# schmidtjonathan/pnmol-experiments

Measured on AMD Instinct MI355X. Metric: filter steps/sec, 1D heat N=512 nu=2 (white-noise EK1 predict+update), higher is better.
Workload: dtype f64; 1 GPU; 1-D heat equation, N=512 mesh, IWP(nu=2) EK1, Dirichlet, dt=2^-7, one problem per GPU (kappa sweep), D=1536, m=514; steps_in_one_call=4975, valid=True, problems_per_gpu=1

## Files before the change

### pnmol-experiments_amd/csrc/pnmol_hip.hip

```cpp
#include <hip/hip_runtime.h>

#include <algorithm>
#include <chrono>
#include <cmath>
#include <cstdio>
#include <cstdlib>
#include <cstring>
#include <string>
#include <utility>
#include <atomic>
#include <vector>

#include "pnmol_hip.h"
#include "pnmol_internal.hpp"

namespace {

constexpr int NB = 32;
constexpr int TLD = NB + 1;
constexpr int MAXN = 4;
typedef double d4 __attribute__((ext_vector_type(4)));

struct IwpConsts {
    double A1[MAXN * MAXN];
    double Q1[MAXN * MAXN];
    double ts[MAXN];
};

struct MeasModel {
    const int* ell_col;
    const double* ell_val;
    int w, d, m, dp, mp;
    double c0, c1;
};

constexpr int HW = 4;

struct HRow {
    int idx[HW + 1];
    double cf[HW + 1];
};

__device__ __forceinline__ void h_row_load(const MeasModel& mm, int i, HRow& r) {
    r.idx[0] = (i < mm.d) ? mm.dp + i : 0;
    r.cf[0] = (i < mm.d) ? mm.c1 : 0.0;
#pragma unroll
    for (int e = 0; e < HW; ++e) {
        const int cidx = (e < mm.w) ? mm.ell_col[e * mm.mp + i] : -1;
        const double val = (e < mm.w) ? mm.ell_val[e * mm.mp + i] : 0.0;
        r.idx[e + 1] = cidx >= 0 ? cidx : 0;
        r.cf[e + 1] = cidx >= 0 ? mm.c0 * val : 0.0;
    }
}

template <typename XT>
__device__ __forceinline__ double h_row_dot(const MeasModel& mm, int i, const XT* x) {
    double v = 0.0;
    if (i < mm.d) v = mm.c1 * x[mm.dp + i];
    for (int e = 0; e < mm.w; ++e) {
        const int cidx = mm.ell_col[e * mm.mp + i];
        if (cidx >= 0) v += mm.c0 * mm.ell_val[e * mm.mp + i] * x[cidx];
    }
    return v;
}

template <int W, typename XT>
__device__ __forceinline__ double h_row_dot_w(const HRow& r, const XT* __restrict__ x) {
    double xv[W + 1];
#pragma unroll
    for (int e = 0; e <= W; ++e) xv[e] = x[r.idx[e]];
    double v = r.cf[0] * xv[0];
#pragma unroll
    for (int e = 1; e <= W; ++e) v += r.cf[e] * xv[e];
    return v;
}

struct RoleArgs {
    IwpConsts c;
    int dp;
    const double* min;
    double* mpred;
    const double* shift;
    double* G;
    double* zbuf;
    MeasModel mm;
    int* flags;
    int nflags;
};

template <int N>
__device__ __forceinline__ void predict_vectors(double* mpl, int tid, const IwpConsts& c, int dp, const double* __restrict__ min,
                                                double* __restrict__ mpred, const double* __restrict__ shift,
                                                double* __restrict__ G, double* __restrict__ zbuf, const MeasModel& mm,
                                                int* __restrict__ flags, int nflags) {
    const long Dp = (long)N * dp;
    for (int e = tid; e < nflags; e += 256) flags[e] = 0;
    for (int j = tid; j < dp; j += 256) {
// ... 1563 lines not shown
                            break;
                        }
                        __builtin_amdgcn_s_sleep(1);
                    }
                }
                __syncthreads();
                const long Dp = (long)RBW * NB;
                const long row0 = (I < zb ? (long)(I - CB) * NB : Dp + (long)(I - zb - 1) * NB) + 8 * w;
                const double* W = F + (long)ld * ld;
                SWEEP_STAMP(2);
                vecops_rowsR<8>(dd.va, W, ld, Dp, row0, row0 + 8, l);
            }
        }
        if (tid == 0 && L.dead) atomicMin(info, -2);
        SWEEP_STAMP(5);
        return;
    }

    SWEEP_STAMP(3);
    if (w == 2 && I > 0) {
        drain_vmem();
        if (l == 0) flag_st(frow + I, I);
        __hip_atomic_store(&L.pub, 1, __ATOMIC_RELAXED, __HIP_MEMORY_SCOPE_WORKGROUP);
    }
    diag4_factor<true>(accD, &L.d4, w, l, F + ((long)I * NB) * ld + (long)I * NB, ld, Linv + (long)I * NB * NB, info, I * NB,
                       L.sd, smax, nullptr, pivot_tolerance(lenient));
    if (w == 1) {
        drain_vmem();
        if (I > 0) {
            int spins = 0;
            while (__hip_atomic_load(&L.pub, __ATOMIC_RELAXED, __HIP_MEMORY_SCOPE_WORKGROUP) == 0 && ++spins < (1 << 24))
                __builtin_amdgcn_s_sleep(1);
        }
        if (l == 0) flag_st(fdiag + I, 1);
        SWEEP_STAMP_L(4);
    }
    if (tid == 0 && L.dead) atomicMin(info, -2);
    if constexpr (CHAINHELP) {
        const int H = CB - 1 - I;
        if (I < H - 1) {
            const double* Xh = F + ((long)H * NB + fr) * ld + 8 * fk;
            for (int t = I + 3; t < H; ++t) {
                const int kh = helper_share(H, t, CB);
                if (kh <= 0) continue;
                int* cl = claim + (long)H * CB + t;
                __syncthreads();
                if (tid == 0) {
                    int got = 0;
                    for (int spins = 0;; ++spins) {
                        if (flag_ld(cl) != 0) break;
                        if (flag_ld(frow + H) >= kh && flag_ld(frow + t) >= kh) {
                            got = atomicCAS(cl, 0, 1) == 0;
                            break;
                        }
                        if (spins > 4096 || flag_ld(fabort)) {
                            got = -1;
                            break;
                        }
                        __builtin_amdgcn_s_sleep(8);
                    }
                    L.seen[0] = got;
                }
                __syncthreads();
                const int got = L.seen[0];
                if (got < 0) break;
                if (got == 0) continue;
                ksplit_partial(L.sP[w], Xh, F + ((long)t * NB + fr) * ld + 8 * fk, 0, kh, ld, w, l);
                __syncthreads();
                double* hs = hs_scratch + ((long)H * CB + t) * NB * NB;
#pragma unroll
                for (int r = 0; r < 4; ++r)
                    wt_st(&hs[(wr * 16 + fk + 4 * r) * NB + colC],
                          (L.sP[0][offC + 4 * r * TLD] + L.sP[1][offC + 4 * r * TLD]) +
                              (L.sP[2][offC + 4 * r * TLD] + L.sP[3][offC + 4 * r * TLD]));
                drain_vmem();
                __syncthreads();
                if (tid == 0) flag_st(cl, 2);
            }
        }
    }
}

constexpr int RL_REP = 8;
constexpr int S_SPLIT_FROM = 11, S_SPLIT_H = 9;
__host__ __device__ inline int s_split_count(int CB, bool xl) { return (xl && CB > S_SPLIT_FROM) ? CB - S_SPLIT_FROM : 0; }
constexpr int W_SPLIT_H = 11;
#ifndef PNMOL_W_SPLIT
#define PNMOL_W_SPLIT 0
#endif
__host__ __device__ inline int w_split_count(int RT, int CB) {
    const int RBW = RT - 2 * CB - 1;
    return (PNMOL_W_SPLIT && RBW > 0 && CB > W_SPLIT_H + 1) ? RBW : 0;
}
struct RlFlags {
    int frow, fabort, fxcc, ffeed, fdiag, fnew, fcol, fdiagL, fnewL, frowL, CBp, total;
};
__host__ __device__ inline RlFlags rl_flags(int RT, int CB) {
    const int RTp = (RT + 31) / 32 * 32, CBp = (CB + 31) / 32 * 32;
    RlFlags f;
    f.CBp = CBp;
    f.frow = 0;
    f.fabort = RTp;
    f.fxcc = RTp + 16;
    f.ffeed = RTp + 32;
    f.fdiag = f.ffeed + CBp;
    f.fnew = f.fdiag + RL_REP * CBp;
    f.fcol = f.fnew + RL_REP * CBp;
    f.fdiagL = f.fcol + RL_REP * CBp;
    f.fnewL = f.fdiagL + CBp;
    f.frowL = f.fnewL + CBp;
    f.total = f.frowL + CBp;
    return f;
}
__device__ __forceinline__ int xcc_id() { return __builtin_amdgcn_s_getreg((3 << 11) | 20) & 15; }
struct WaveWait {
    bool dead;
};
__device__ __forceinline__ void wave_wait_ge(const int* p, int need, int* fabort, WaveWait& ww) {
    if (ww.dead) return;
    for (int spins = 0;; ++spins) {
        if (flag_ld(p) >= need) return;
        if (spins > SWEEP_SPIN_LIMIT || ((spins & 63) == 63 && flag_ld(fabort))) {
            ww.dead = true;
            flag_st(fabort, 1);
            return;
        }
        __builtin_amdgcn_s_sleep(1);
    }
}
__device__ __forceinline__ void relay_wait_ge(const int* p, int need, int* relay, int tag, int* fabort, WaveWait& ww, int w) {
    if (w == 0) {
        wave_wait_ge(p, need, fabort, ww);
        __hip_atomic_store(relay, ww.dead ? (1 << 30) : tag, __ATOMIC_RELAXED, __HIP_MEMORY_SCOPE_WORKGROUP);
    } else {
        int v;
        while ((v = __hip_atomic_load(relay, __ATOMIC_RELAXED, __HIP_MEMORY_SCOPE_WORKGROUP)) < tag) __builtin_amdgcn_s_sleep(1);
        if (v == (1 << 30)) ww.dead = true;
    }
    asm volatile("" ::: "memory");
}

template <class Need>
__device__ __forceinline__ void relay_progress(const int* p, int cnt, Need need, int want, int& known, int* relay, int* fabort,
                                               WaveWait& ww, int w, int l) {
    if (w == 0) {
        if (known < want) {
            for (int spins = 0; !ww.dead; ++spins) {
                const int v = l < cnt ? flag_ld(p + l) : 0;
                const unsigned long long ok = __ballot(l < cnt && v >= need(l));
                known = __builtin_amdgcn_readfirstlane((int)__builtin_ctzll(~ok));
                if (known >= want) break;
                if (spins > SWEEP_SPIN_LIMIT || ((spins & 63) == 63 && flag_ld(fabort))) {
                    ww.dead = true;
                    flag_st(fabort, 1);
                    break;
                }
                __builtin_amdgcn_s_sleep(1);
            }
            __hip_atomic_store(relay, ww.dead ? (1 << 30) : known, __ATOMIC_RELAXED, __HIP_MEMORY_SCOPE_WORKGROUP);
        }
    } else {
        int v;
        while ((v = __hip_atomic_load(relay, __ATOMIC_RELAXED, __HIP_MEMORY_SCOPE_WORKGROUP)) < want) __builtin_amdgcn_s_sleep(1);
        if (v == (1 << 30)) ww.dead = true;
    }
    asm volatile("" ::: "memory");
}
__device__ __forceinline__ void relay_progress_min(const int* p, int cnt, int want, int& known, int* relay, int* fabort,
                                                   WaveWait& ww, int w, int l) {
    if (w == 0) {
        if (known < want) {
            for (int spins = 0; !ww.dead; ++spins) {
                int v = l < cnt ? flag_ld(p + l) : (1 << 29);
#pragma unroll
                for (int o = 32; o > 0; o >>= 1) v = min(v, __shfl_xor(v, o));
                known = __builtin_amdgcn_readfirstlane(v);
// ... 170 lines not shown
        if (XL && w == 1 && J + 1 < CB) {
            TileRegs t1;
            tile_regs_from_lds(t1, C.sLinv, l);
            tile_regs_store<0>(t1, rlinv, (unsigned)(J * NB * NB * 8), NB, l);
            drain_vmem();
            if (l == 0) l2_flag_st(rflags, fl.fdiagL + J, 1);
        }
        if (J + 1 == CB) {
            __syncthreads();
            if (w == 2) {
                wt_rows_from_lds<8>(rlinv, (unsigned)(J * NB * NB * 8), NB, C.sLinv, 0, l);
                drain_vmem();
                if (l < RL_REP) flag_st(fdiag_all + l * CBp + J, 1);
                if (XL && l == 0) l2_flag_st(rflags, fl.fdiagL + J, 1);
            }
            break;
        }
        if (w == 0 || w == 2) {
            wave_wait_ge(ffeed + J + 1, 1, fabort, ww);
            sc1_tile_to_lds((w == 2) ? C.sFeedD : C.sFeedS, rfeed, (unsigned)((2 * (J + 1) + (w == 2 ? 1 : 0)) * NB * NB * 8), l);
            if (w == 2 && l < NB) C.sd[(J + 1) & 1][l] = G[(long)((J + 1) * NB + l) * ld + (J + 1) * NB + l];
        }
        __syncthreads();
        CHAIN_TRACE(J, 2);
        if (tid < 16) C.d4[(J + 1) & 1].flagA[tid] = 0;
        TileRegs tl;
        if (w == 2) {
            if constexpr (XL) {
                tile_regs_from_lds(tl, C.sLinv, l);
            } else {
                wt_rows_from_lds<8>(rlinv, (unsigned)(J * NB * NB * 8), NB, C.sLinv, 0, l);
            }
        }
        d4 x = {0, 0, 0, 0};
#pragma unroll
        for (int s = 0; s < 8; ++s)
            x = __builtin_amdgcn_mfma_f64_16x16x4f64(C.sFeedS[(wr * 16 + fr) * TLD + 8 * fk + s],
                                                     C.sLinv[(wc * 16 + fr) * TLD + 8 * fk + s], x, 0, 0, 0);
#pragma unroll
        for (int r = 0; r < 4; ++r) C.sX[offC + 4 * r * TLD] = x[r];
#pragma unroll
        for (int r = 0; r < 4; ++r) accD[r] = C.sFeedD[offC + 4 * r * TLD];
        __syncthreads();
        CHAIN_TRACE(J, 3);
        if (w == 2) {
            if constexpr (!XL) {
                drain_vmem();
                if (l < RL_REP) flag_st(fdiag_all + l * CBp + J, 1);
            }
        }
#pragma unroll
        for (int s = 0; s < 8; ++s)
            accD = __builtin_amdgcn_mfma_f64_16x16x4f64(C.sX[(wr * 16 + fr) * TLD + 8 * fk + s],
                                                        C.sX[(wc * 16 + fr) * TLD + 8 * fk + s], accD, 0, 0, 0);
        if (w == 2) {
            const unsigned orgX = (unsigned)((((long)(J + 1) * NB) * ld + (long)J * NB) * 8);
            if constexpr (XL) {
                TileRegs tx;
                tile_regs_from_lds(tx, C.sX, l);
                tile_regs_store<0>(tx, rF, orgX, ld, l);
                drain_vmem();
                if (l == 0) l2_flag_st(rflags, fl.fnewL + J, 1);
                tile_regs_store<16>(tl, rlinv, (unsigned)(J * NB * NB * 8), NB, l);
                tile_regs_store<16>(tx, rF, orgX, ld, l);
                drain_vmem();
                if (l < RL_REP) flag_st(fdiag_all + l * CBp + J, 1);
                if (l < RL_REP) flag_st(fnew_all + l * CBp + J, 1);
            } else {
                wt_rows_from_lds<8>(rF, orgX, ld, C.sX, 0, l);
                drain_vmem();
                if (l < RL_REP) flag_st(fnew_all + l * CBp + J, 1);
            }
        }
    }
    if (w == 2)
        diag4_output(&C.d4[(CB - 1) & 1], l, F + ((long)(CB - 1) * NB) * ld + (long)(CB - 1) * NB, ld, info, (CB - 1) * NB,
                     C.sd[(CB - 1) & 1], smax, pivtol);
    if (l == 0 && ww.dead) atomicMin(info, -2);
}

template <int N, bool FUSED, int MAXT, bool XL>
__global__ __launch_bounds__(256) void k_sweep_rl(const double* __restrict__ G, double* F, double* Linv, int ld, int CB,
                                                  int RT, int* flags, int* info_base, const int* __restrict__ ctr,
                                                  DowndateArgs dd, double* feed, int lenient, int home) {
    __shared__ __attribute__((aligned(16))) union {
        SweepLds L;
        ChainLds C;
    } lds;
    SweepLds& L = lds.L;
    __shared__ __attribute__((aligned(16))) double bulk_ring[4][RING + 2][16 * NB];
    const int tid = threadIdx.x, l = tid & 63, w = __builtin_amdgcn_readfirstlane(tid >> 6);
    const int wr = w >> 1, wc = w & 1, fr = l & 15, fk = l >> 4;
    const RlFlags fl = rl_flags(RT, CB);
    int* frow = flags + fl.frow;
    int* fabort = flags + fl.fabort;
    int* ffeed = flags + fl.ffeed;
    const int* fdiag = flags + fl.fdiag + (blockIdx.x % RL_REP) * fl.CBp;
    const int* fnew = flags + fl.fnew + (blockIdx.x % RL_REP) * fl.CBp;
    const int* fcol = flags + fl.fcol + (blockIdx.x % RL_REP) * fl.CBp;
    int* info = info_base + (*ctr - 1);
    const int bx = XL ? (int)blockIdx.x - home : (int)blockIdx.x;
    if (bx < 0) return;
    if (bx == 0) {
        sweep_chain_role<XL>(lds.C, G, F, Linv, ld, CB, flags, fl, info, feed, lenient, tid, l, w);
        return;
    }
    int I, part = 0;
    if constexpr (XL) {
        const int nsplit = s_split_count(CB, true);
        const int b = bx, nslot = 8 * (CB - 1 + nsplit) + 1;
        if (b < nslot) {
            if (b % 8 != 0) return;
            const int sidx = b / 8;
            if (sidx < CB) {
                I = sidx;
                part = (nsplit > 0 && I >= S_SPLIT_FROM) ? 1 : 0;
            } else {
                I = S_SPLIT_FROM + (sidx - CB);
                part = 2;
            }
        } else {
            if (b % 8 == 0) return;
            const int q = b - nslot;
            I = CB + q - (q + 1) / 8;
        }
    } else {
        I = bx - 1;
    }
#ifdef PNMOL_SWEEP_STAMP
    if (tid == 0) L.stamp_id = part == 1 ? 200 + I : 1 + I;
#endif
    {
        const int zb = RT - CB - 1;
        if (I >= CB && I <= zb) I = (I == CB) ? zb : I - 1;
    }
    const int nwsplit = w_split_count(RT, CB);
    if (I >= RT && I < RT + nwsplit) {
        I = CB + (I - RT);
        part = 2;
    } else if (I >= RT) {
        I -= nwsplit;
        if constexpr (FUSED) {
            if (tid == 0) {
                L.dead = 0, L.seen[0] = 0;
                __builtin_amdgcn_fence(__ATOMIC_ACQUIRE, "agent");
            }
            __syncthreads();
            SWEEP_STAMP(0);
            sweep_downdate_role<N, true>(L, dd, F, ld, CB, CB, frow, fabort, info, I - RT, tid, l, w, *ctr - 1);
        }
        return;
    } else if (nwsplit > 0 && I >= CB && I < RT - CB - 1) {
        part = 1;
    }
    const bool chain = I < CB;
    if (chain && I == 0) return;
    if (tid == 0) {
        L.dead = 0, L.pub = 0, L.pubcnt = part == 2 ? 4 * (I < CB ? S_SPLIT_H : W_SPLIT_H) : 0, L.rdiag = 0, L.rnew = 0, L.rcol = 0, L.rzb = 0;
        L.seen[0] = 0;
        __builtin_amdgcn_fence(__ATOMIC_ACQUIRE, "agent");
    }
    __syncthreads();
    SWEEP_STAMP(0);

    const long rowC = (long)I * NB + wr * 16 + fk;
    const int colC = wc * 16 + fr;
    const int offC = (wr * 16 + fk) * TLD + colC;
    const bool feeds = chain && part != 1;
    const int hsplit = chain ? S_SPLIT_H : W_SPLIT_H;
    const int t0 = part == 2 ? hsplit : 0;
    const int last = part == 1 ? hsplit - 1 : (chain ? I - 2 : CB - 1);
    const int ntiles = part == 1 ? hsplit : (chain ? I : CB);
    d4 n[MAXT];
#pragma unroll
    for (int t = 0; t < MAXT; ++t)
        if (t0 + t < ntiles) {
#pragma unroll
            for (int r = 0; r < 4; ++r) n[t][r] = -G[(rowC + 4 * r) * ld + (long)(t0 + t) * NB + colC];
        }
    d4 accD = {0, 0, 0, 0};
    if (feeds) {
#pragma unroll
        for (int r = 0; r < 4; ++r) {
            const int rl = wr * 16 + fk + 4 * r, cl = colC;
            accD[r] = -G[((long)I * NB + (rl >= cl ? rl : cl)) * ld + (long)I * NB + (rl >= cl ? cl : rl)];
        }
    }
    WaveWait ww{false};
    int known_diag = 0, known_new = 0, known_col = 0;
    const __amdgpu_buffer_rsrc_t rF = wt_rsrc(F), rfeed = wt_rsrc(feed), rflags = wt_rsrc(flags);
    const double* ringw = &bulk_ring[w][0][0];
    const unsigned ring0 = __builtin_amdgcn_readfirstlane((unsigned)(size_t)ringw);
    int roff[4], roffL[4];
#pragma unroll
    for (int c = 0; c < 4; ++c) {
        const int row = 4 * c + (l >> 4);
        roff[c] = (wc * 16 + row) * ld + 2 * ((l & 15) ^ row);
        roffL[c] = (wc * 16 + row) * NB + 2 * ((l & 15) ^ row);
    }
#ifndef PNMOL_EAGER_TILES
#define PNMOL_EAGER_TILES 6
#endif
    constexpr int EAGER_TILES = PNMOL_EAGER_TILES;
    bool pre_b0 = false;
    if constexpr (FUSED) {
        const int RBW = RT - 2 * CB - 1, zb = CB + RBW;
        if (!chain && I > zb) {
            double bq[8] = {0, 0, 0, 0, 0, 0, 0, 0};
            if (dd.va.Sqinv != nullptr) rows8_dot(dd.va.Sqinv, (long)(I - zb - 1) * NB + 8 * w, ld, dd.va.z, bq, l);
            if (l == 0) {
#pragma unroll
                for (int q = 0; q < 8; ++q) L.sd[8 * w + q] = bq[q];
            }
        }
    }
    bool local = false;
    if constexpr (XL) {
        if (chain) {
            if (tid == 0) {
                int v = 0;
                for (int spins = 0; spins < 4096 && (v = flag_ld(flags + fl.fxcc)) == 0; ++spins) __builtin_amdgcn_s_sleep(1);
                L.seen[0] = (v == 1 + xcc_id());
            }
            __syncthreads();
            local = L.seen[0] != 0;
            if (local) fdiag = flags + fl.fdiagL, fnew = flags + fl.fnewL;
        }
    }
    Frag8 ax;
    auto flag_tile = [&](int t) {
        drain_vmem();
        int lastw = 0;
        if (l == 0) lastw = __hip_atomic_fetch_add(&L.pubcnt, 1, __ATOMIC_RELAXED, __HIP_MEMORY_SCOPE_WORKGROUP) == 4 * t + 3;
        if (__builtin_amdgcn_readfirstlane(lastw)) {
            if (l == 0) flag_st(frow + I, t + 1);
            if (XL && chain && l == 0) {
                if (local) l2_flag_st(rflags, fl.frowL + I, t + 1);
                else flag_st(flags + fl.frowL + I, t + 1);
            }
            if (chain && l < RL_REP)
                __hip_atomic_fetch_add(flags + fl.fcol + l * fl.CBp + t, 1, __ATOMIC_RELAXED, __HIP_MEMORY_SCOPE_AGENT);
        }
    };
    if (part == 2) {
        const int* fsrc = (XL && local) ? flags + fl.frowL : frow;
        for (int k = 0; k < t0; ++k) {
            if (chain) {
                if (k + 1 < t0) {
                    relay_progress_min(fsrc + t0, I - t0 + 1, k + 1, known_col, &L.rcol, fabort, ww, w, l);
                } else {
                    relay_progress(fnew, CB - 1, [](int) { return 1; }, t0, known_new, &L.rnew, fabort, ww, w, l);
                    relay_progress_min(fsrc + t0 + 1, I - t0, t0, known_col, &L.rcol, fabort, ww, w, l);
                }
            } else {
                relay_progress(fnew, CB - 1, [](int) { return 1; }, k + 1, known_new, &L.rnew, fabort, ww, w, l);
                relay_progress(fcol, CB - 1, [CB](int q) { return CB - 2 - q; }, k + 1, known_col, &L.rcol, fabort, ww, w, l);
                relay_wait_ge(frow + I, k + 1, &L.rzb, k + 1, fabort, ww, w);
            }
            Frag8 bx;
            frag_ld(ax, F + ((long)I * NB + wr * 16 + fr) * ld + (long)k * NB + 8 * fk);
            frag_ld(bx, F + ((long)I * NB + wc * 16 + fr) * ld + (long)k * NB + 8 * fk);
#pragma unroll
            for (int u0 = 0; u0 < 8; u0 += 4) {
                Frag8 b[4];
#pragma unroll
                for (int q = 0; q < 4; ++q)
                    if (t0 + u0 + q < ntiles)
                        frag_ld(b[q], F + ((long)(t0 + u0 + q) * NB + wc * 16 + fr) * ld + (long)k * NB + 8 * fk);
#pragma unroll
                for (int q = 0; q < 4; ++q)
                    if (t0 + u0 + q < ntiles) {
#pragma unroll
                        for (int s = 0; s < 8; ++s)
                            n[u0 + q] = __builtin_amdgcn_mfma_f64_16x16x4f64(ax.v[s], b[q].v[s], n[u0 + q], 0, 0, 0);
                    }
            }
            if (chain) {
#pragma unroll
                for (int s = 0; s < 8; ++s) accD = __builtin_amdgcn_mfma_f64_16x16x4f64(ax.v[s], bx.v[s], accD, 0, 0, 0);
            }
            mfma_result_guard();
        }
    }
    const bool lastlocal = feeds && XL && local;
#pragma unroll
    for (int r = 0; r < 4; ++r) L.sS[t0 & 1][offC + 4 * r * TLD] = -n[0][r];
    __syncthreads();
    bool pre_l = false;
    for (int j = t0; j <= last; ++j) {
// ... 244 lines not shown
        }
#pragma unroll
        for (int a = 0; a < N; ++a) {
            st[(a * 16 + lr) * C::SLD + lc] = pa[a].x;
            st[(a * 16 + lr) * C::SLD + lc + 1] = pa[a].y;
            st[((N + a) * 16 + lr) * C::SLD + lc] = pb[a].x;
            st[((N + a) * 16 + lr) * C::SLD + lc + 1] = pb[a].y;
        }
        asm volatile("" ::: "memory");
        __builtin_amdgcn_wave_barrier();
#pragma unroll
        for (int kk = 0; kk < C::CW / 4; ++kk) {
            double fa[N], fb[N];
#pragma unroll
            for (int a = 0; a < N; ++a) {
                fa[a] = st[(a * 16 + fr) * C::SLD + kk * 4 + fk];
                fb[a] = st[((N + a) * 16 + fr) * C::SLD + kk * 4 + fk];
            }
#pragma unroll
            for (int a = 0; a < N; ++a)
#pragma unroll
                for (int b = 0; b < N; ++b)
                    acc[a][b] = __builtin_amdgcn_mfma_f64_16x16x4f64(fa[a], fb[b], acc[a][b], 0, 0, 0);
        }
        asm volatile("" ::: "memory");
        __builtin_amdgcn_wave_barrier();
    }
    __syncthreads();
    if (w >= 2) {
        double* rd = smem + (w - 2) * C::RED;
#pragma unroll
        for (int a = 0; a < N; ++a)
#pragma unroll
            for (int b = 0; b < N; ++b)
#pragma unroll
                for (int r = 0; r < 4; ++r) rd[((a * N + b) * 4 + r) * 64 + l] = acc[a][b][r];
    }
    __syncthreads();
    if (w >= 2) return;
    {
        const double* rd = smem + w * C::RED;
#pragma unroll
        for (int a = 0; a < N; ++a)
#pragma unroll
            for (int b = 0; b < N; ++b)
#pragma unroll
                for (int r = 0; r < 4; ++r) acc[a][b][r] += rd[((a * N + b) * 4 + r) * 64 + l];
    }
    __syncthreads();
    if (w == 0)
        downdate_finish<N, 0>(acc, smem, Ppred, Pout, var, dp, Dp, J, K, l);
    else
        downdate_finish<N, 1>(acc, smem, Ppred, Pout, var, dp, Dp, J, K, l);
}

__global__ __launch_bounds__(256) void k_fill_q(void* __restrict__ Qf, const double* __restrict__ Kg, IwpConsts c, int n,
                                                int dp, int p32) {
    const long Dp = (long)n * dp;
    const long e = (long)blockIdx.x * 256 + threadIdx.x;
    if (e >= Dp * Dp) return;
    const long row = e / Dp, col = e % Dp;
    const int a = (int)(row / dp), j = (int)(row % dp), b = (int)(col / dp), k = (int)(col % dp);
    const double v = c.Q1[a * MAXN + b] * Kg[(long)j * dp + k];
    if (p32) static_cast<float*>(Qf)[e] = (float)v;
    else static_cast<double*>(Qf)[e] = v;
}

__global__ __launch_bounds__(256) void k_ttt(const double* __restrict__ T, double* __restrict__ C, int mp) {
    __shared__ double sa[16][17], sb[16][17];
    const int tx = threadIdx.x & 15, ty = threadIdx.x >> 4;
    const int i = blockIdx.y * 16 + ty, k = blockIdx.x * 16 + tx;
    double acc = 0.0;
    for (int q0 = 0; q0 < mp; q0 += 16) {
        sa[ty][tx] = T[(long)(blockIdx.y * 16 + ty) * mp + q0 + tx];
        sb[ty][tx] = T[(long)(blockIdx.x * 16 + ty) * mp + q0 + tx];
        __syncthreads();
#pragma unroll
        for (int q = 0; q < 16; ++q) acc += sa[ty][q] * sb[tx][q];
        __syncthreads();
    }
    C[(long)i * mp + k] = acc;
}

template <int N, bool ROLE>
__global__ __launch_bounds__(256) void k_readout(const double* __restrict__ mean, const double* __restrict__ var,
                                                 double* __restrict__ means_base, double* __restrict__ stds_base,
                                                 double s0, int d, const double* __restrict__ part,
                                                 double* __restrict__ rec_base, int mp, int* __restrict__ ctr,
                                                 RoleArgs ra, int* __restrict__ tickets, int rblocks,
                                                 const void* __restrict__ Ppred, const double* __restrict__ rdiag,
                                                 const double* __restrict__ Rdense, int p32) {
    if constexpr (ROLE) {
        if ((int)blockIdx.x > rblocks) {
            const int fb = blockIdx.x - rblocks - 1;
            if (p32) front_block_tiled(static_cast<const float*>(Ppred), ra.G, rdiag, Rdense, ra.mm, (long)N * ra.dp, fb);
            else front_block_tiled(static_cast<const double*>(Ppred), ra.G, rdiag, Rdense, ra.mm, (long)N * ra.dp, fb);
            return;
        }
    }
    const int slot = __builtin_amdgcn_readfirstlane(*ctr) - 1;
    if constexpr (ROLE) {
        if ((int)blockIdx.x == rblocks) {
            extern __shared__ double mpl[];
            predict_vectors<N>(mpl, threadIdx.x, ra.c, ra.dp, ra.min, ra.mpred, ra.shift, ra.G, ra.zbuf, ra.mm, ra.flags,
                               ra.nflags);
            if (threadIdx.x == 0) {
                int spins = 0;
                while (__hip_atomic_load(tickets, __ATOMIC_RELAXED, __HIP_MEMORY_SCOPE_AGENT) < rblocks &&
                       ++spins < (1 << 22)) __builtin_amdgcn_s_sleep(1);
                *ctr = slot + 2;
                __hip_atomic_store(tickets, 0, __ATOMIC_RELAXED, __HIP_MEMORY_SCOPE_AGENT);
            }
            return;
        }
        __syncthreads();
        if (threadIdx.x == 0) atomicAdd(tickets, 1);
    }
    const int j = blockIdx.x * blockDim.x + threadIdx.x;
    double* means = means_base ? means_base + (size_t)slot * d : nullptr;
    double* stds = stds_base ? stds_base + (size_t)slot * d : nullptr;
    double* rec = rec_base + 4 * (size_t)slot;
    if (j < d) {
        if (means) means[j] = s0 * mean[j];
        if (stds) stds[j] = s0 * sqrt(fmax(var[j], 0.0));
    }
    if (blockIdx.x == 0) {
        __shared__ double sred[3][4];
        double a[3] = {0.0, 0.0, 0.0};
        for (int i = threadIdx.x; i < mp; i += 256)
#pragma unroll
            for (int q = 0; q < 3; ++q) a[q] += part[q * mp + i];
#pragma unroll
        for (int q = 0; q < 3; ++q)
#pragma unroll
            for (int o = 32; o > 0; o >>= 1) a[q] += __shfl_xor(a[q], o);
        if ((threadIdx.x & 63) == 0)
            for (int q = 0; q < 3; ++q) sred[q][threadIdx.x >> 6] = a[q];
        __syncthreads();
        if (threadIdx.x < 3) rec[threadIdx.x] = sred[threadIdx.x][0] + sred[threadIdx.x][1] + sred[threadIdx.x][2] + sred[threadIdx.x][3];
    }
}

__global__ __launch_bounds__(256) void k_poison(double* __restrict__ F, long nF, double* __restrict__ Linv, long nL,
                                                double* __restrict__ hs, long nH) {
    const double bad = __longlong_as_double(0x7ff8dead0000beefLL);
    const long stride = (long)gridDim.x * 256;
    for (long e = (long)blockIdx.x * 256 + threadIdx.x; e < nF; e += stride) F[e] = bad;
    for (long e = (long)blockIdx.x * 256 + threadIdx.x; e < nL; e += stride) {
        const int r = (int)((e / NB) % NB), c = (int)(e % NB);
        if (!(r < 16 && c >= 16)) Linv[e] = bad;
    }
    for (long e = (long)blockIdx.x * 256 + threadIdx.x; e < nH; e += stride) hs[e] = bad;
}

__global__ void k_operator_diagonal(double* __restrict__ ell_val, const double* __restrict__ base_val,
                                    const int* __restrict__ slot, const double* __restrict__ op ,
                                    double* __restrict__ shift, int d, int mp) {
    const int i = blockIdx.x * blockDim.x + threadIdx.x;
    if (i >= mp) return;
    if (i < d) {
        const int e = slot[i];
        ell_val[(long)e * mp + i] = base_val[(long)e * mp + i] - op[i];
    }
    shift[i] = op[d + i];
}

constexpr int FD_MAXS = 16;
__global__ __launch_bounds__(128) void k_fd_solve(const double* __restrict__ gram, const double* __restrict__ dk,
                                                  const double* __restrict__ llk, int N, int s, double* __restrict__ w,
                                                  double* __restrict__ unc) {
    const int p = blockIdx.x * blockDim.x + threadIdx.x;
    if (p >= N) return;
    double A[FD_MAXS][FD_MAXS], b[FD_MAXS];
    for (int i = 0; i < s; ++i) {
        for (int k = 0; k < s; ++k) A[i][k] = gram[((long)p * s + i) * s + k];
        b[i] = dk[(long)p * s + i];
    }
    for (int c = 0; c < s; ++c) {
        int piv = c;
        double best = fabs(A[c][c]);
        for (int i = c + 1; i < s; ++i)
            if (fabs(A[i][c]) > best) best = fabs(A[i][c]), piv = i;
        if (piv != c) {
            for (int k = 0; k < s; ++k) {
                const double t = A[c][k];
                A[c][k] = A[piv][k], A[piv][k] = t;
            }
            const double t = b[c];
            b[c] = b[piv], b[piv] = t;
        }
        const double inv = 1.0 / A[c][c];
        for (int i = c + 1; i < s; ++i) {
            const double f = A[i][c] * inv;
            A[i][c] = f;
            for (int k = c + 1; k < s; ++k) A[i][k] -= f * A[c][k];
        }
    }
    for (int i = 1; i < s; ++i)
        for (int k = 0; k < i; ++k) b[i] -= A[i][k] * b[k];
    for (int i = s - 1; i >= 0; --i) {
        for (int k = i + 1; k < s; ++k) b[i] -= A[i][k] * b[k];
        b[i] /= A[i][i];
    }
    double dot = 0.0;
    for (int i = 0; i < s; ++i) {
        w[(long)p * s + i] = b[i];
        dot += b[i] * dk[(long)p * s + i];
    }
    unc[p] = llk[p] - dot;
}

#define HIPCHK(ctx, call)                                                                        \
    do {                                                                                         \
        hipError_t e__ = (call);                                                                 \
// ... 206 lines not shown
    IwpConsts iwp{};
    int* ell_col = nullptr;
    double* ell_val = nullptr;
    int* ell_col_base = nullptr;
    double* ell_val_base = nullptr;
    int* ell_diag_slot = nullptr;
    int base_w = 0, base_has_diag = 0;
    int ell_is_base = 1;
    double* h_op = nullptr;
    double* h_op_dev = nullptr;
    hipEvent_t ev_op = nullptr;
    double *Kg = nullptr, *rdiag = nullptr, *Rdense = nullptr, *shift = nullptr;
    double *G = nullptr, *F = nullptr, *Linv = nullptr, *Ppred = nullptr, *mpred = nullptr, *zbuf = nullptr;
    double *var = nullptr, *Sqinv = nullptr, *rec = nullptr, *part = nullptr, *sdiag = nullptr;
    int* info = nullptr;
    std::vector<double> sqdiag;
    double* Qfull = nullptr;
    int* one = nullptr;
    int* info_err = nullptr;
    double sq_dt = -1.0;
    std::vector<double> hB;
    int ell_cap = 0;
    double *tmpP = nullptr, *tmpMean = nullptr;
    double *rec_means = nullptr, *rec_stds = nullptr;
    double* h_pin = nullptr;
    double* h_pin_dev = nullptr;
    int rec_cap = 0;
    hipEvent_t ev0 = nullptr, ev1 = nullptr;
    float last_ms = 0.f;
    int* ctr = nullptr;
    int pending_k = 0;
    double pending_dt = 0.0;
    pnmol_state* pending_state = nullptr;
    struct GraphEntry {
        double *P0, *P1, *var;
        double dt;
        int nsteps;
        bool have_sq;
        bool fused;
        hipGraphExec_t exec;
        bool launched;
    };
    std::vector<GraphEntry> graphs;
    int graph_chunk = 10;

};

struct pnmol_state {
    pnmol_filter* f = nullptr;
    double* mean = nullptr;
    double* P = nullptr;
    double* var = nullptr;
    double t = 0.0;
    double frame_dt = 0.0;
};

namespace {

void drop_graphs(pnmol_filter* f);

enum StepKind { STEP_FULL = 0, STEP_FIRST = 1, STEP_STEADY = 2 };

inline bool fused_loop(const pnmol_filter* f) { return f->sweep_mode == 2 && f->n <= 3 && f->fuse_predict != 0; }

inline bool sweep_rl_enabled() {
    static const int on = [] {
        const char* e = std::getenv("PNMOL_HIP_SWEEP_RL");
        return e ? std::atoi(e) : 1;
    }();
    return on != 0;
}
inline int sweep_xl_mode() {
    static const int mode = [] {
        const char* e = std::getenv("PNMOL_HIP_SWEEP_XL");
        return e ? (std::atoi(e) != 0 ? 1 : 0) : -1;
    }();
    return mode;
}
constexpr int MAX_DEVICES = 64;
std::atomic<int> live_rl_filters[MAX_DEVICES];
template <int N, bool FUSED>
void launch_sweep(unsigned grid, hipStream_t st, const double* G, double* F, double* Linv, int ld, int CB, int RT, int* flags,
                  int* info, const int* ctr, const DowndateArgs& dd, int* claim, double* hs, int lenient, int home,
                  bool wskip = false) {
    const bool xl = home >= 0;
    const unsigned rgrid = grid + (unsigned)w_split_count(RT, CB);
    unsigned xgrid = 8u * (unsigned)(CB - 1 + s_split_count(CB, true)) + 1u;
    for (unsigned left = rgrid - (unsigned)CB; left > 0; ++xgrid)
        if (xgrid % 8u != 0u) --left;
    xgrid += (unsigned)(xl ? home : 0);
    if (sweep_rl_enabled() && CB <= 9) {
        if (xl) k_sweep_rl<N, FUSED, 9, true><<<xgrid, 256, 0, st>>>(G, F, Linv, ld, CB, RT, flags, info, ctr, dd, hs, lenient, home);
        else k_sweep_rl<N, FUSED, 9, false><<<rgrid + 1, 256, 0, st>>>(G, F, Linv, ld, CB, RT, flags, info, ctr, dd, hs, lenient, home);
    } else if (sweep_rl_enabled() && CB <= 17) {
        if (xl) k_sweep_rl<N, FUSED, 17, true><<<xgrid, 256, 0, st>>>(G, F, Linv, ld, CB, RT, flags, info, ctr, dd, hs, lenient, home);
        else k_sweep_rl<N, FUSED, 17, false><<<rgrid + 1, 256, 0, st>>>(G, F, Linv, ld, CB, RT, flags, info, ctr, dd, hs, lenient, home);
    }
    else
        k_sweep<N, FUSED><<<grid, 256, 0, st>>>(G, F, Linv, ld, CB, RT, flags, info, ctr, dd, claim, hs, lenient, wskip ? 1 : 0);
}

inline bool short_last_panel() {
    static const int on = [] {
        const char* e = std::getenv("PNMOL_HIP_SHORT_LAST");
        return e ? std::atoi(e) : 1;
    }();
    return on != 0;
}
template <int N>
int launch_step(pnmol_filter* f, const double* Pin, const double* min, double frame_dt, double dt, double* Pout,
                double* mout, double* varout, bool record, StepKind kind) {
    pnmol_ctx* ctx = f->ctx;
    hipStream_t st = ctx->stream;
    IwpConsts c = f->iwp;
    for (int a = 0; a < f->n; ++a) {
        const double so = frame_dt == 0.0 ? 1.0 : nordsieck_scale(f->nu, a, frame_dt);
        c.ts[a] = so / nordsieck_scale(f->nu, a, dt);
    }
    MeasModel mm{f->ell_col, f->ell_val, f->ellw, f->d, f->m, f->dp, f->mp,
                 nordsieck_scale(f->nu, 0, dt), nordsieck_scale(f->nu, 1, dt)};
    const int dp = f->dp, mp = f->mp;
    const long Dp = f->Dp;

    if (kind != STEP_STEADY)
        k_predict<N><<<dim3(dp / 32, dp / 8 + 1), dim3(32, 8), sizeof(double) * Dp, st>>>(
        Pin, f->Ppred, f->Kg, c, dp, min, f->mpred, f->shift, f->G, f->zbuf, mm, f->ctr, f->flags, f->nflags, f->p32);
    if (kind != STEP_STEADY) {
        if (f->ellw > HW && f->sweep_mode != 0) {
            k_front<<<dim3((mp + 255) / 256, (unsigned)Dp), 256, 0, st>>>(f->Ppred, f->G, f->rdiag, f->Rdense, mm, Dp, f->p32);
            k_front_s<<<dim3((mp + 255) / 256, (unsigned)mp), 256, 0, st>>>(f->G, f->rdiag, f->Rdense, mm);
        } else {
            k_front<<<dim3((mp + 255) / 256, (unsigned)(Dp + mp + (f->sweep_mode == 0 ? mp : 0))), 256, 0, st>>>(
                f->Ppred, f->G, f->rdiag, f->Rdense, mm, Dp, f->p32);
        }
    }
    const long rowI0 = (long)mp + Dp + NB;
    const double* W = f->F + (long)mp * mp;
    const bool have_sq = (f->Sqinv != nullptr && f->sq_dt == dt);
    VecArgs va{f->mpred, f->F + ((long)mp + Dp) * mp, f->F + rowI0 * mp, f->zbuf, have_sq ? f->Sqinv : nullptr,
               mout, f->part};
    const int nreal = f->m - NB * (f->CB - 1);
    DowndateArgs dd{f->Ppred, Pout, varout, dp, 0, va, kind == STEP_FULL ? nullptr : f->Ppred, f->Kg, f->last_ctr, {}, {}, f->p32,
                    (nreal < 8 && short_last_panel()) ? nreal : 0};
    std::memcpy(dd.A1, f->iwp.A1, sizeof(dd.A1));
    std::memcpy(dd.Q1, f->iwp.Q1, sizeof(dd.Q1));
    if (f->sweep_mode == 2) {
        const int t32 = dp / NB, pairs = t32 * (t32 + 1) / 2;
        dd.vrows = 0;
        if constexpr (N <= 3)
            launch_sweep<N, true>(f->RT + pairs, st, f->G, f->F, f->Linv, mp, f->CB, f->RT, f->flags, f->info, f->ctr, dd,
                                  f->flags + f->RT + f->CB + 1, f->hs_scratch, f->p32 ? 2 : 0, f->xcd_home);
    } else {
        if (f->sweep_mode == 1) {
            if (f->w_gemm) {
                launch_sweep<N, false>(2 * f->CB + 1, st, f->G, f->F, f->Linv, mp, f->CB, f->RT, f->flags, f->info, f->ctr, dd,
                                       f->flags + f->RT + f->CB + 1, f->hs_scratch, f->p32 ? 2 : 0, f->xcd_home, true);
                const int nI = (int)(Dp / BDT), nt = nI * (mp / BDT);
                k_w_gemm<<<8 * ((nt + 7) / 8), 256, 0, st>>>(f->G + (long)mp * mp, f->F + rowI0 * mp, f->F + (long)mp * mp, mp, nI, nt);
            } else
            launch_sweep<N, false>(f->RT, st, f->G, f->F, f->Linv, mp, f->CB, f->RT, f->flags, f->info, f->ctr, dd,
                                   f->flags + f->RT + f->CB + 1, f->hs_scratch, f->p32 ? 2 : 0, f->xcd_home);
        } else {
            k_diag0<<<1, 128, 0, st>>>(f->G, f->F, f->Linv, mp, f->info, f->sdiag, f->ctr);
            for (int j = 0; j < f->CB; ++j) {
                const int nrb = f->RT - (j + 1);
                const int ncb = f->CB - 1 - j > 0 ? f->CB - 1 - j : 1;
                k_panel<<<dim3(nrb, ncb), 256, 0, st>>>(f->G, f->F, f->Linv, mp, j, f->CB, f->RBS, f->info, f->sdiag, f->ctr);
            }
        }
        const int tiles = dp / 16;
        const int vrows = (int)(((Dp + mp + 3) / 4 + tiles - 1) / tiles);
        if (f->dd_big) {
            const int T = (int)(Dp / BDT), nt = T * (T + 1) / 2;
            if (f->p32)
                k_downdate_big<float><<<8 * ((nt + 7) / 8), 256, 0, st>>>(reinterpret_cast<const float*>(f->Ppred), W,
                                                                          reinterpret_cast<float*>(Pout), varout, Dp, mp, nt);
            else
                k_downdate_big<double><<<8 * ((nt + 7) / 8), 256, 0, st>>>(static_cast<const double*>(f->Ppred), W, Pout, varout,
                                                                           Dp, mp, nt);
            k_vecops<<<dim3(tiles, vrows), 256, 0, st>>>(va, W, mp, Dp, tiles);
        } else {
            k_downdate<N><<<dim3(tiles, tiles + vrows), 256, 0, st>>>(f->Ppred, W, Pout, varout, dp, mp, 0, mp / 8, va);
        }
    }
    IwpConsts cn = f->iwp;
    for (int a = 0; a < MAXN; ++a) cn.ts[a] = 1.0;
    RoleArgs ra{cn, dp, mout, f->mpred, f->shift, f->G, f->zbuf, mm, f->flags, f->nflags};
    const unsigned rblocks = (f->d + 255) / 256;
    if (kind == STEP_FULL)
        k_readout<N, false><<<rblocks, 256, 0, st>>>(mout, varout, record ? f->rec_means : nullptr,
                                                    record ? f->rec_stds : nullptr, nordsieck_scale(f->nu, 0, dt), f->d,
                                                    f->part, f->rec, mp, f->ctr, ra, f->tickets, (int)rblocks, f->Ppred, f->rdiag,
                                                    f->Rdense, f->p32);
    else
        k_readout<N, true><<<rblocks + 1 + (unsigned)front_tiled_blocks(Dp, mp), 256, sizeof(double) * Dp, st>>>(
            mout, varout, record ? f->rec_means : nullptr, record ? f->rec_stds : nullptr, nordsieck_scale(f->nu, 0, dt),
            f->d, f->part, f->rec, mp, f->ctr, ra, f->tickets, (int)rblocks, f->Ppred, f->rdiag, f->Rdense, f->p32);
    hipError_t e = hipGetLastError();
    if (e != hipSuccess) {
        ctx->err = std::string("kernel launch: ") + hipGetErrorString(e);
        return -2;
    }
    return 0;
}

int dispatch_step(pnmol_filter* f, const double* Pin, const double* min, double frame_dt, double dt, double* Pout,
                  double* mout, double* varout, bool record, StepKind kind = STEP_FULL) {
    switch (f->n) {
        case 2: return launch_step<2>(f, Pin, min, frame_dt, dt, Pout, mout, varout, record, kind);
        case 3: return launch_step<3>(f, Pin, min, frame_dt, dt, Pout, mout, varout, record, kind);
        case 4: return launch_step<4>(f, Pin, min, frame_dt, dt, Pout, mout, varout, record, kind);
    }
    return -1;
}

void drop_graphs(pnmol_filter* f) {
    for (auto& g : f->graphs)
        if (g.exec) (void)hipGraphExecDestroy(g.exec);
    f->graphs.clear();
}

int get_graph(pnmol_filter* f, double* P0, double* M0, double* P1, double* M1, double* var, double dt, int nsteps,
              hipGraphExec_t* out) {
    pnmol_ctx* ctx = f->ctx;
    const bool have_sq = (f->Sqinv != nullptr && f->sq_dt == dt);
    for (auto& g : f->graphs)
        if (g.P0 == P0 && g.P1 == P1 && g.var == var && g.dt == dt && g.nsteps == nsteps && g.have_sq == have_sq &&
            g.fused == fused_loop(f)) {
            *out = g.exec;
            return 0;
        }
    if (f->graphs.size() >= 8) drop_graphs(f);
    hipGraph_t graph = nullptr;
    HIPCHK(ctx, hipStreamBeginCapture(ctx->stream, hipStreamCaptureModeThreadLocal));
    int rc = 0;
    for (int it = 0; it < nsteps && rc == 0; ++it)
        rc = (it & 1) ? dispatch_step(f, P1, M1, dt, dt, P0, M0, var, true, fused_loop(f) ? STEP_STEADY : STEP_FULL)
                      : dispatch_step(f, P0, M0, dt, dt, P1, M1, var, true, fused_loop(f) ? STEP_STEADY : STEP_FULL);
    hipError_t e = hipStreamEndCapture(ctx->stream, &graph);
    if (rc != 0 || e != hipSuccess) {
        if (graph) (void)hipGraphDestroy(graph);
        if (rc == 0) ctx->err = std::string("hipStreamEndCapture: ") + hipGetErrorString(e);
        return rc != 0 ? rc : -2;
    }
    hipGraphExec_t exec = nullptr;
    e = hipGraphInstantiate(&exec, graph, nullptr, nullptr, 0);
    (void)hipGraphDestroy(graph);
    if (e != hipSuccess) {
        ctx->err = std::string("hipGraphInstantiate: ") + hipGetErrorString(e);
        return -2;
    }
    f->graphs.push_back({P0, P1, var, dt, nsteps, have_sq, fused_loop(f), exec, false});
    *out = exec;
    return 0;
}

int build_ell(const double* M, const double* B, int d, int ds, int nB, int mp, std::vector<int>& ecol,
              std::vector<double>& eval) {
    const int m = d + nB;
    int w = 1;
    for (int i = 0; i < m; ++i) {
        int c = 0;
        const double* row = i < d ? M + (long)i * ds : B + (long)(i - d) * ds;
        for (int k = 0; k < ds; ++k) c += row[k] != 0.0;
        w = c > w ? c : w;
    }
    ecol.assign((size_t)w * mp, -1);
    eval.assign((size_t)w * mp, 0.0);
    for (int i = 0; i < m; ++i) {
        int e = 0;
        for (int k = 0; k < ds; ++k) {
            const double v = i < d ? -M[(long)i * ds + k] : B[(long)(i - d) * ds + k];
            if (v != 0.0) {
                ecol[(size_t)e * mp + i] = k;
                eval[(size_t)e * mp + i] = v;
                ++e;
            }
        }
    }
    return w;
// ... 1164 lines not shown
```

Baseline: 8071 steps/s.

## Drop last-stage sweep blocks, fold Q1 back-substitution into readout, refill home XCD slots

Adds a 'nolst' mode that launches CB fewer sweep blocks and copies z into part at the zb row. The dropped residual/quadratic-form work is recomputed in the readout kernel's block 0 by a block-triangular back-substitution through F and Linv in LDS. It also factors the XL block-to-row mapping into a layout header and lets non-critical tiles fill spare slots on the home XCD, shrinking the grid. The aim is to take the last-stage tiles off the sweep's critical path and use idle home-XCD slots. The cost is a serial back-substitution in one readout block plus extra dynamic LDS.

Result: slower. 7864 steps/s (median of 2 runs) (-2.6%).

```diff
diff --git a/pnmol-experiments_amd/csrc/pnmol_hip.hip b/pnmol-experiments_amd/csrc/pnmol_hip.hip
--- a/pnmol-experiments_amd/csrc/pnmol_hip.hip
+++ b/pnmol-experiments_amd/csrc/pnmol_hip.hip
@@ -13,6 +13,7 @@
 
 #include "pnmol_hip.h"
 #include "pnmol_internal.hpp"
+#include "sweep_layout.hpp"
 
 namespace {
 
@@ -1742,16 +1743,11 @@
 }
 
 constexpr int RL_REP = 8;
-constexpr int S_SPLIT_FROM = 11, S_SPLIT_H = 9;
-__host__ __device__ inline int s_split_count(int CB, bool xl) { return (xl && CB > S_SPLIT_FROM) ? CB - S_SPLIT_FROM : 0; }
-constexpr int W_SPLIT_H = 11;
-#ifndef PNMOL_W_SPLIT
-#define PNMOL_W_SPLIT 0
-#endif
-__host__ __device__ inline int w_split_count(int RT, int CB) {
-    const int RBW = RT - 2 * CB - 1;
-    return (PNMOL_W_SPLIT && RBW > 0 && CB > W_SPLIT_H + 1) ? RBW : 0;
-}
+using pnmol_layout::S_SPLIT_FROM;
+using pnmol_layout::S_SPLIT_H;
+using pnmol_layout::W_SPLIT_H;
+using pnmol_layout::s_split_count;
+using pnmol_layout::w_split_count;
 struct RlFlags {
     int frow, fabort, fxcc, ffeed, fdiag, fnew, fcol, fdiagL, fnewL, frowL, CBp, total;
 };
@@ -2088,7 +2084,8 @@
 template <int N, bool FUSED, int MAXT, bool XL>
 __global__ __launch_bounds__(256) void k_sweep_rl(const double* __restrict__ G, double* F, double* Linv, int ld, int CB,
                                                   int RT, int* flags, int* info_base, const int* __restrict__ ctr,
-                                                  DowndateArgs dd, double* feed, int lenient, int home) {
+                                                  DowndateArgs dd, double* feed, int lenient, int home, int nolst,
+                                                  int fill) {
     __shared__ __attribute__((aligned(16))) union {
         SweepLds L;
         ChainLds C;
@@ -2111,11 +2108,13 @@
         sweep_chain_role<XL>(lds.C, G, F, Linv, ld, CB, flags, fl, info, feed, lenient, tid, l, w);
         return;
     }
+    const int RTe = nolst ? RT - CB : RT;
+    const int nwsplit = w_split_count(RT, CB, XL && nolst);
     int I, part = 0;
     if constexpr (XL) {
         const int nsplit = s_split_count(CB, true);
-        const int b = bx, nslot = 8 * (CB - 1 + nsplit) + 1;
-        if (b < nslot) {
+        const int b = bx;
+        if (b < pnmol_layout::xl_first_slot(CB)) {
             if (b % 8 != 0) return;
             const int sidx = b / 8;
             if (sidx < CB) {
@@ -2126,9 +2125,9 @@
                 part = 2;
             }
         } else {
-            if (b % 8 == 0) return;
-            const int q = b - nslot;
-            I = CB + q - (q + 1) / 8;
+            const int q = pnmol_layout::xl_noncritical_index(b, CB, fill);
+            if (q < 0) return;
+            I = CB + q;
         }
     } else {
         I = bx - 1;
@@ -2140,12 +2139,11 @@
         const int zb = RT - CB - 1;
         if (I >= CB && I <= zb) I = (I == CB) ? zb : I - 1;
     }
-    const int nwsplit = w_split_count(RT, CB);
-    if (I >= RT && I < RT + nwsplit) {
-        I = CB + (I - RT);
+    if (I >= RTe && I < RTe + nwsplit) {
+        I = CB + (I - RTe);
         part = 2;
-    } else if (I >= RT) {
-        I -= nwsplit;
+    } else if (I >= RTe) {
+        I -= nwsplit + RTe - RT;
         if constexpr (FUSED) {
             if (tid == 0) {
                 L.dead = 0, L.seen[0] = 0;
@@ -2211,6 +2209,8 @@
     bool pre_b0 = false;
     if constexpr (FUSED) {
         const int RBW = RT - 2 * CB - 1, zb = CB + RBW;
+        if (nolst && I == zb)
+            for (int i = tid; i < ld; i += 256) dd.va.part[ld + i] = dd.va.z[i];
         if (!chain && I > zb) {
             double bq[8] = {0, 0, 0, 0, 0, 0, 0, 0};
             if (dd.va.Sqinv != nullptr) rows8_dot(dd.va.Sqinv, (long)(I - zb - 1) * NB + 8 * w, ld, dd.va.z, bq, l);
@@ -2621,6 +2621,60 @@
     C[(long)i * mp + k] = acc;
 }
 
+struct Q1Args {
+    const double* F;
+    const double* Linv;
+    const double* r;
+    const double* z;
+};
+__device__ __forceinline__ void q1_backsub(const Q1Args& q, int mp, double* acc , double* xs ,
+                                           int tid) {
+    const int CB = mp / NB;
+    for (int i = tid; i < mp; i += 256) acc[i] = q.z[i];
+    double lv[NB];
+    if (tid < NB) {
+#pragma unroll
+        for (int r = 0; r < NB; ++r) lv[r] = q.Linv[(long)(CB - 1) * NB * NB + r * NB + tid];
+    }
+    __syncthreads();
+    for (int J = CB - 1; J >= 0; --J) {
+        const int ncol = J * NB;
+        double u0[NB], u1[NB];
+        if (ncol > 0) {
+            const double* Lr = q.F + (long)J * NB * mp;
+            const int c0 = tid < ncol ? tid : ncol - 1, c1 = tid + 256 < ncol ? tid + 256 : ncol - 1;
+#pragma unroll
+            for (int r = 0; r < NB; ++r) {
+                u0[r] = Lr[(long)r * mp + c0];
+                u1[r] = Lr[(long)r * mp + c1];
+            }
+        }
+        if (tid < NB) {
+            double x = 0.0;
+#pragma unroll
+            for (int r = 0; r < NB; ++r) x += (r >= tid ? lv[r] : 0.0) * acc[J * NB + r];
+            xs[J * NB + tid] = x;
+            if (J > 0) {
+#pragma unroll
+                for (int r = 0; r < NB; ++r) lv[r] = q.Linv[(long)(J - 1) * NB * NB + r * NB + tid];
+            }
+        }
+        __syncthreads();
+        if (ncol > 0) {
+            double a0 = 0.0, a1 = 0.0;
+#pragma unroll
+            for (int r = 0; r < NB; ++r) {
+                const double xr = xs[J * NB + r];
+                a0 += u0[r] * xr;
+                a1 += u1[r] * xr;
+            }
+            if (tid < ncol) acc[tid] -= a0;
+            if (tid + 256 < ncol) acc[tid + 256] -= a1;
+        }
+        __syncthreads();
+    }
+}
+
 template <int N, bool ROLE>
 __global__ __launch_bounds__(256) void k_readout(const double* __restrict__ mean, const double* __restrict__ var,
                                                  double* __restrict__ means_base, double* __restrict__ stds_base,
@@ -2628,7 +2682,7 @@
                                                  double* __restrict__ rec_base, int mp, int* __restrict__ ctr,
                                                  RoleArgs ra, int* __restrict__ tickets, int rblocks,
                                                  const void* __restrict__ Ppred, const double* __restrict__ rdiag,
-                                                 const double* __restrict__ Rdense, int p32) {
+                                                 const double* __restrict__ Rdense, int p32, Q1Args q1) {
     if constexpr (ROLE) {
         if ((int)blockIdx.x > rblocks) {
             const int fb = blockIdx.x - rblocks - 1;
@@ -2666,9 +2720,18 @@
     if (blockIdx.x == 0) {
         __shared__ double sred[3][4];
         double a[3] = {0.0, 0.0, 0.0};
-        for (int i = threadIdx.x; i < mp; i += 256)
-#pragma unroll
-            for (int q = 0; q < 3; ++q) a[q] += part[q * mp + i];
+        if (q1.F) {
+            extern __shared__ double q1s[];
+            q1_backsub(q1, mp, q1s, q1s + mp, threadIdx.x);
+            for (int i = threadIdx.x; i < mp; i += 256) {
+                a[0] += __dmul_rn(q1.r[i], q1.r[i]);
+                a[1] += __dmul_rn(q1s[mp + i], q1s[mp + i]);
+            }
+        } else {
+            for (int i = threadIdx.x; i < mp; i += 256)
+#pragma unroll
+                for (int q = 0; q < 3; ++q) a[q] += part[q * mp + i];
+        }
 #pragma unroll
         for (int q = 0; q < 3; ++q)
 #pragma unroll
@@ -3041,19 +3104,21 @@
 template <int N, bool FUSED>
 void launch_sweep(unsigned grid, hipStream_t st, const double* G, double* F, double* Linv, int ld, int CB, int RT, int* flags,
                   int* info, const int* ctr, const DowndateArgs& dd, int* claim, double* hs, int lenient, int home,
-                  bool wskip = false) {
+                  bool wskip = false, bool nolst = false) {
     const bool xl = home >= 0;
-    const unsigned rgrid = grid + (unsigned)w_split_count(RT, CB);
-    unsigned xgrid = 8u * (unsigned)(CB - 1 + s_split_count(CB, true)) + 1u;
-    for (unsigned left = rgrid - (unsigned)CB; left > 0; ++xgrid)
-        if (xgrid % 8u != 0u) --left;
-    xgrid += (unsigned)(xl ? home : 0);
+    nolst = nolst && FUSED && sweep_rl_enabled() && CB <= 17;
+    if (nolst) grid -= (unsigned)CB;
+    const unsigned rgrid = grid + (unsigned)w_split_count(RT, CB, xl && nolst);
+    const int count = (int)rgrid - CB;
+    const int fill = xl ? pnmol_layout::xl_home_fill(CB, count) : 0;
+    const unsigned xgrid = (unsigned)pnmol_layout::xl_grid(CB, count) + (unsigned)(xl ? home : 0);
+    const int nl = nolst ? 1 : 0;
     if (sweep_rl_enabled() && CB <= 9) {
-        if (xl) k_sweep_rl<N, FUSED, 9, true><<<xgrid, 256, 0, st>>>(G, F, Linv, ld, CB, RT, flags, info, ctr, dd, hs, lenient, home);
-        else k_sweep_rl<N, FUSED, 9, false><<<rgrid + 1, 256, 0, st>>>(G, F, Linv, ld, CB, RT, flags, info, ctr, dd, hs, lenient, home);
+        if (xl) k_sweep_rl<N, FUSED, 9, true><<<xgrid, 256, 0, st>>>(G, F, Linv, ld, CB, RT, flags, info, ctr, dd, hs, lenient, home, nl, fill);
+        else k_sweep_rl<N, FUSED, 9, false><<<rgrid + 1, 256, 0, st>>>(G, F, Linv, ld, CB, RT, flags, info, ctr, dd, hs, lenient, home, nl, 0);
     } else if (sweep_rl_enabled() && CB <= 17) {
-        if (xl) k_sweep_rl<N, FUSED, 17, true><<<xgrid, 256, 0, st>>>(G, F, Linv, ld, CB, RT, flags, info, ctr, dd, hs, lenient, home);
-        else k_sweep_rl<N, FUSED, 17, false><<<rgrid + 1, 256, 0, st>>>(G, F, Linv, ld, CB, RT, flags, info, ctr, dd, hs, lenient, home);
+        if (xl) k_sweep_rl<N, FUSED, 17, true><<<xgrid, 256, 0, st>>>(G, F, Linv, ld, CB, RT, flags, info, ctr, dd, hs, lenient, home, nl, fill);
+        else k_sweep_rl<N, FUSED, 17, false><<<rgrid + 1, 256, 0, st>>>(G, F, Linv, ld, CB, RT, flags, info, ctr, dd, hs, lenient, home, nl, 0);
     }
     else
         k_sweep<N, FUSED><<<grid, 256, 0, st>>>(G, F, Linv, ld, CB, RT, flags, info, ctr, dd, claim, hs, lenient, wskip ? 1 : 0);
@@ -3098,6 +3163,8 @@
     const bool have_sq = (f->Sqinv != nullptr && f->sq_dt == dt);
     VecArgs va{f->mpred, f->F + ((long)mp + Dp) * mp, f->F + rowI0 * mp, f->zbuf, have_sq ? f->Sqinv : nullptr,
                mout, f->part};
+    const bool q1bs = N <= 3 && f->sweep_mode == 2 && !have_sq && sweep_rl_enabled() && f->CB <= 17;
+    const Q1Args q1{q1bs ? f->F : nullptr, f->Linv, f->F + ((long)mp + Dp) * mp, f->part + mp};
     const int nreal = f->m - NB * (f->CB - 1);
     DowndateArgs dd{f->Ppred, Pout, varout, dp, 0, va, kind == STEP_FULL ? nullptr : f->Ppred, f->Kg, f->last_ctr, {}, {}, f->p32,
                     (nreal < 8 && short_last_panel()) ? nreal : 0};
@@ -3108,7 +3175,7 @@
         dd.vrows = 0;
         if constexpr (N <= 3)
             launch_sweep<N, true>(f->RT + pairs, st, f->G, f->F, f->Linv, mp, f->CB, f->RT, f->flags, f->info, f->ctr, dd,
-                                  f->flags + f->RT + f->CB + 1, f->hs_scratch, f->p32 ? 2 : 0, f->xcd_home);
+                                  f->flags + f->RT + f->CB + 1, f->hs_scratch, f->p32 ? 2 : 0, f->xcd_home, false, q1bs);
     } else {
         if (f->sweep_mode == 1) {
             if (f->w_gemm) {
@@ -3147,14 +3214,15 @@
     RoleArgs ra{cn, dp, mout, f->mpred, f->shift, f->G, f->zbuf, mm, f->flags, f->nflags};
     const unsigned rblocks = (f->d + 255) / 256;
     if (kind == STEP_FULL)
-        k_readout<N, false><<<rblocks, 256, 0, st>>>(mout, varout, record ? f->rec_means : nullptr,
+        k_readout<N, false><<<rblocks, 256, q1bs ? sizeof(double) * 2 * mp : 0, st>>>(mout, varout, record ? f->rec_means : nullptr,
                                                     record ? f->rec_stds : nullptr, nordsieck_scale(f->nu, 0, dt), f->d,
                                                     f->part, f->rec, mp, f->ctr, ra, f->tickets, (int)rblocks, f->Ppred, f->rdiag,
-                                                    f->Rdense, f->p32);
+                                                    f->Rdense, f->p32, q1);
     else
-        k_readout<N, true><<<rblocks + 1 + (unsigned)front_tiled_blocks(Dp, mp), 256, sizeof(double) * Dp, st>>>(
+        k_readout<N, true><<<rblocks + 1 + (unsigned)front_tiled_blocks(Dp, mp), 256,
+                             sizeof(double) * std::max(Dp, q1bs ? 2L * mp : 0L), st>>>(
             mout, varout, record ? f->rec_means : nullptr, record ? f->rec_stds : nullptr, nordsieck_scale(f->nu, 0, dt),
-            f->d, f->part, f->rec, mp, f->ctr, ra, f->tickets, (int)rblocks, f->Ppred, f->rdiag, f->Rdense, f->p32);
+            f->d, f->part, f->rec, mp, f->ctr, ra, f->tickets, (int)rblocks, f->Ppred, f->rdiag, f->Rdense, f->p32, q1);
     hipError_t e = hipGetLastError();
     if (e != hipSuccess) {
         ctx->err = std::string("kernel launch: ") + hipGetErrorString(e);
diff --git a/pnmol-experiments_amd/csrc/sweep_layout.hpp b/pnmol-experiments_amd/csrc/sweep_layout.hpp
--- /dev/null
+++ b/pnmol-experiments_amd/csrc/sweep_layout.hpp
@@ -0,0 +1,40 @@
+#pragma once
+
+#if !defined(__HIPCC__) && !defined(__host__)
+#define __host__
+#define __device__
+#endif
+
+namespace pnmol_layout {
+
+constexpr int S_SPLIT_FROM = 11, S_SPLIT_H = 9;
+__host__ __device__ inline int s_split_count(int CB, bool xl) { return (xl && CB > S_SPLIT_FROM) ? CB - S_SPLIT_FROM : 0; }
+
+constexpr int W_SPLIT_H = 11;
+__host__ __device__ inline int w_split_count(int RT, int CB, bool on) {
+    const int RBW = RT - 2 * CB - 1;
+    return (on && RBW > 0 && CB > W_SPLIT_H + 1) ? RBW : 0;
+}
+
+__host__ __device__ inline int xl_home_critical(int CB) { return CB + s_split_count(CB, true); }
+__host__ __device__ inline int xl_first_slot(int CB) { return 8 * (xl_home_critical(CB) - 1) + 1; }
+__host__ __device__ inline int xl_home_fill(int CB, int count) {
+    const int spare = 32 - xl_home_critical(CB), need = count - 7 * 32;
+    return need <= 0 || spare <= 0 ? 0 : (need < spare ? need : spare);
+}
+__host__ __device__ inline int xl_noncritical_index(int b, int CB, int fill) {
+    const int d = b - xl_first_slot(CB);
+    if (d < 0) return -1;
+    if ((d + 1) % 8 == 0 && (d + 1) / 8 > fill) return -1;
+    const int h = d / 8;
+    return d - (h > fill ? h - fill : 0);
+}
+__host__ __device__ inline int xl_grid(int CB, int count) {
+    const int fill = xl_home_fill(CB, count);
+    int b = xl_first_slot(CB);
+    for (int left = count; left > 0; ++b)
+        if (xl_noncritical_index(b, CB, fill) >= 0) --left;
+    return b;
+}
+
+}
```
